# biod/sambamba

Measured on NVIDIA H100. Metric: bam_gb_per_s_depth_base, higher is better.
Workload: dtype u32

## Files before the change

__graft_entry__.py:

```python
import os
import subprocess
import sys

ROOT = os.path.dirname(os.path.abspath(__file__))
CSRC = os.path.join(ROOT, "sambamba_b200", "csrc")
NVCC = os.environ.get("NVCC", "/usr/local/cuda/bin/nvcc")


def _run(cmd, cwd=None, quiet=False):
    r = subprocess.run(cmd, cwd=cwd, stdout=subprocess.PIPE, stderr=subprocess.STDOUT, text=True)
    if r.returncode != 0:
        sys.stderr.write(r.stdout)
        raise RuntimeError("build step failed: " + " ".join(cmd))
    if not quiet and r.stdout.strip():
        print(r.stdout.strip()[-2000:])


def _stale(target, sources):
    if not os.path.exists(target):
        return True
    t = os.path.getmtime(target)
    return any(os.path.getmtime(s) > t for s in sources if os.path.exists(s))


def build(quiet=False, load=True):
    out = os.path.join(ROOT, "sambamba_b200", "_build")
    os.makedirs(out, exist_ok=True)
    lib = os.path.join(out, "libbdepth.so")
    srcs = [os.path.join(CSRC, f) for f in ("bdepth.cu", "kernels.cuh", "mates.cuh", "filter.cuh", "regex.cuh", "host_filter.hpp", "host_regex.hpp", "launch.cuh", "inflate_core.cuh", "inflate2_core.cuh", "host_bam.hpp")] + [os.path.join(ROOT, "include", "bdepth.h"), os.path.abspath(__file__)]
    if _stale(lib, srcs):
        _run([NVCC, "-gencode", "arch=compute_90a,code=sm_90a", "-O3", "-lineinfo", "-std=c++17",
              "-Xcompiler", "-fPIC,-Wall,-Wno-unused-function,-Wno-unknown-pragmas", "-shared", "-o", lib, os.path.join(CSRC, "bdepth.cu"), "-lcudart", "-ldl"], quiet=quiet)
    cli_src = os.path.join(CSRC, "cli.cpp")
    cli = os.path.join(out, "sambamba-depth-b200")
    if os.path.exists(cli_src) and _stale(cli, [cli_src, lib]):
        _run(["g++", "-O2", "-g", "-std=c++17", "-Wall", "-o", cli, cli_src, "-L" + out, "-lbdepth", "-Wl,-rpath,$ORIGIN"], quiet=quiet)
    _run(["make", "-s", "-C", os.path.join(ROOT, "oracle")], quiet=quiet)
    tb = os.path.join(ROOT, "tools", "_build")
    os.makedirs(tb, exist_ok=True)
    if _stale(os.path.join(tb, "bamgen"), [os.path.join(ROOT, "tools", "bamgen.c")]):
        _run(["gcc", "-O2", "-g", "-o", os.path.join(tb, "bamgen"), os.path.join(ROOT, "tools", "bamgen.c"), "-lz", "-lpthread", "-lm"], quiet=quiet)
    fso = os.path.join(ROOT, "tools", "flagstat_oracle.c")
    if _stale(os.path.join(tb, "flagstat_oracle"), [fso]) or _stale(os.path.join(tb, "libflagstat_oracle.so"), [fso]):
        _run(["gcc", "-O2", "-g", "-Wall", "-std=gnu11", "-DORACLE_MAIN", "-o", os.path.join(tb, "flagstat_oracle"), fso, "-lz", "-lpthread"], quiet=quiet)
        _run(["gcc", "-O2", "-g", "-Wall", "-std=gnu11", "-fPIC", "-shared", "-o", os.path.join(tb, "libflagstat_oracle.so"), fso, "-lz", "-lpthread"], quiet=quiet)
    vco = os.path.join(ROOT, "tools", "view_count_oracle.c")
    if _stale(os.path.join(tb, "view_count_oracle"), [vco]) or _stale(os.path.join(tb, "libview_count_oracle.so"), [vco]):
        _run(["gcc", "-O2", "-g", "-Wall", "-std=gnu11", "-DORACLE_MAIN", "-o", os.path.join(tb, "view_count_oracle"), vco, "-lz", "-lm"], quiet=quiet)
        _run(["gcc", "-O2", "-g", "-Wall", "-std=gnu11", "-fPIC", "-shared", "-o", os.path.join(tb, "libview_count_oracle.so"), vco, "-lz", "-lm"], quiet=quiet)
    _run(["make", "-s", "-C", os.path.join(ROOT, "tests", "emul")], quiet=quiet)
    emul = os.path.join(ROOT, "tests", "emul")
    es = os.path.join(emul, "libemul_sam.so")
    es_srcs = [os.path.join(emul, f) for f in ("emul_sam.cpp", "cuda_shim.cpp", "cuda_shim.hpp")] + [os.path.join(CSRC, f) for f in ("kernels.cuh", "filter.cuh", "regex.cuh", "launch.cuh", "inflate_core.cuh", "inflate2_core.cuh")]
    if _stale(es, es_srcs):
        _run(["g++", "-O2", "-g", "-std=c++17", "-w", "-DBDEPTH_EMULATE_SHIM=\"" + os.path.join(emul, "cuda_shim.hpp") + "\"", "-shared", "-fPIC", "-o", es,
              os.path.join(emul, "emul_sam.cpp"), os.path.join(emul, "cuda_shim.cpp"), "-ldl"], quiet=quiet)
    if load:
        sys.path.insert(0, ROOT)
        import sambamba_b200
        sambamba_b200.load_library()


def smoke():
    sys.path.insert(0, ROOT)
    sys.path.insert(0, os.path.join(ROOT, "tests"))
    import numpy as np
    import sambamba_b200 as sb
    import helpers
    path = os.path.join(ROOT, "tests", "golden", "issue_204.bam")
    win = helpers.interesting_window(path)
    with sb.BDepth(path, device=0) as b:
        got = b.run_base(window=win)
        st = b.stats()
    want, _ = helpers.oracle_counts(path, window=win)
    assert got.shape == want.shape and np.array_equal(got, want), "GPU counters differ from the oracle"
    print("smoke ok:", {k: st[k] for k in ("n_blocks", "n_records", "n_records_pass", "covered_positions", "gpu_launches")})


if __name__ == "__main__":
    build()
    if len(sys.argv) > 1 and sys.argv[1] == "smoke":
        smoke()
```

sambamba_b200/csrc/bdepth.cu:

```cuda
#include "launch.cuh"
#include <dlfcn.h>
#include <fcntl.h>
#include <stdarg.h>
#include <stdio.h>
#include <stdlib.h>
#include <sys/mman.h>
#include <sys/stat.h>
#include <unistd.h>
#include <algorithm>
#include <chrono>
#include <map>
#include <string>
#include <vector>

#include "../../include/bdepth.h"
#include "host_bam.hpp"
#include "kernels.cuh"
#include "mates.cuh"
#include "host_filter.hpp"

using namespace bdk;

namespace {

// ... 46 lines not shown
enum RunMode { RUN_FULL = 0, RUN_INFLATE_ONLY = 1, RUN_SCAN_ONLY = 2, RUN_INDEX = 3, RUN_FLAGSTAT = 4, RUN_VIEW_COUNT = 5, RUN_VIEW_TEXT = 6 };
constexpr int RC_RETRY_WINDOW = 1;

struct NcclUid { char b[128]; };
typedef void* NcclComm;
struct NcclApi {
    bool ok = false; std::string err;
    int (*GetUniqueId)(NcclUid*) = nullptr;
    int (*CommInitRank)(NcclComm*, int, NcclUid, int) = nullptr;
    int (*CommDestroy)(NcclComm) = nullptr;
    int (*AllGather)(const void*, void*, size_t, int, NcclComm, cudaStream_t) = nullptr;
    int (*AllReduce)(const void*, void*, size_t, int, int, NcclComm, cudaStream_t) = nullptr;
    int (*Send)(const void*, size_t, int, int, NcclComm, cudaStream_t) = nullptr;
    int (*Recv)(void*, size_t, int, int, NcclComm, cudaStream_t) = nullptr;
    int (*GroupStart)() = nullptr;
    int (*GroupEnd)() = nullptr;
    const char* (*GetErrorString)(int) = nullptr;
};
constexpr int NCCL_UINT32 = 3, NCCL_UINT64 = 5, NCCL_SUM = 0;
NcclApi& nccl() {
    static NcclApi api; static bool tried = false;
    if (tried) return api;
    tried = true;
#ifdef BDEPTH_EMULATE_SHIM
    api.GetUniqueId = [](NcclUid* u) { return emu_ncclGetUniqueId(u->b); };
    api.CommInitRank = [](NcclComm* c, int w, NcclUid u, int r) { return emu_ncclCommInitRank(c, w, u.b, r); };
    api.CommDestroy = emu_ncclCommDestroy; api.AllGather = emu_ncclAllGather; api.AllReduce = emu_ncclAllReduce; api.Send = emu_ncclSend; api.Recv = emu_ncclRecv;
    api.GroupStart = emu_ncclGroupStart; api.GroupEnd = emu_ncclGroupEnd; api.GetErrorString = emu_ncclGetErrorString; api.ok = true;
    return api;
#endif
    void* lib = dlopen("libnccl.so.2", RTLD_NOW | RTLD_GLOBAL);
    if (!lib) lib = dlopen("libnccl.so", RTLD_NOW | RTLD_GLOBAL);
    if (!lib) { api.err = std::string("cannot load libnccl.so.2: ") + dlerror(); return api; }
    bool all = true;
    auto sym = [&](const char* n) { void* p = dlsym(lib, n); if (!p) { all = false; api.err = std::string("missing NCCL symbol ") + n; } return p; };
    api.GetUniqueId = (int (*)(NcclUid*))sym("ncclGetUniqueId");
    api.CommInitRank = (int (*)(NcclComm*, int, NcclUid, int))sym("ncclCommInitRank");
    api.CommDestroy = (int (*)(NcclComm))sym("ncclCommDestroy");
    api.AllGather = (int (*)(const void*, void*, size_t, int, NcclComm, cudaStream_t))sym("ncclAllGather");
    api.AllReduce = (int (*)(const void*, void*, size_t, int, int, NcclComm, cudaStream_t))sym("ncclAllReduce");
    api.Send = (int (*)(const void*, size_t, int, int, NcclComm, cudaStream_t))sym("ncclSend");
    api.Recv = (int (*)(void*, size_t, int, int, NcclComm, cudaStream_t))sym("ncclRecv");
    api.GroupStart = (int (*)())sym("ncclGroupStart");
    api.GroupEnd = (int (*)())sym("ncclGroupEnd");
    api.GetErrorString = (const char* (*)(int))sym("ncclGetErrorString");
    api.ok = all;
    return api;
}

}

struct bdepth {
    const uint8_t* file = nullptr; size_t file_len = 0; bool mapped = false; int fd = -1;
    std::vector<HostBlock> blocks; uint64_t total_u = 0;
    bool lazy = false, framed_all = true; size_t framed_off = 0;
    BamHeader hdr; BaiIndex bai; bool has_index = false;
    int device = 0; int n_sm = 0;
    int mapq_gt = 0; uint32_t flag_reject = 0x600; uint32_t minq = 0;
    std::vector<bdepth_region> regions;
    int rank = 0, world = 1;
    NcclComm comm = nullptr; bool have_uid = false; NcclUid uid{};
    uint64_t own_lo = 0, own_hi = 0;
    bool bai_window_ok = true;
    bool combined = false;
    bool fix_mates = false;
    bool k1lz_v12 = false;
    bool k1lz_flat = false;
    int k1h_variant = -1;
    bool k1_onephase = false;
    bool k3_pre = false;
    bool k3_tile = true;
    bool has_fprog = false; FilterProg fprog; DevBuf fprog_d;
    DevBuf m_hash, m_flag, m_flt, m_ctl;
    uint32_t S = 1;
    DevBuf rg_ids, rg_offs, rg_samp;
    DevBuf text[2], text_tiles, text_offs, text_zero, text_samp, present;
    int coll_pending = 0;
    bool want_presence = false;
    uint64_t batch_u = 6ull << 30;
    uint64_t chunk_blocks = 13 * 32 * 16;
    bool shard_ready = false;
    size_t blk_lo = 0, blk_hi = 0; int64_t entry0 = 0; uint64_t limit_abs_u = 0;
    uint64_t zone_lin_lo = UINT64_MAX;
    uint64_t own_lo_abs_u = 0;
    bool sparse_ok = true;
    bool sparse_on = false;
    std::vector<HostBlock> vblocks; std::vector<int32_t> seg_entry ; std::vector<uint32_t> seg_limit ;
    DevBuf anchors_idx, anchors_val, chunk_limit;
    cudaStream_t s_main = nullptr, s_copy = nullptr, s_d2h = nullptr;
    cudaEvent_t ev[32] = {};
    DevBuf comp2[2];
    cudaStream_t s_k1[16] = {};
    std::vector<cudaEvent_t> chunk_ev[2], k1_ev;
    std::vector<size_t> chunk_end[2];
    bool staged = false; uint64_t staged_file_off = 0;
    DevBuf tok, lits, aux, segi, littab;
    DevBuf comp, descs, status, ubuf, chunk_start, entry, exitb, count, slot_base, slots, rec_base, walk_list;
    DevBuf soa_start, soa_span, soa_meta, soa_off, soa_ncl, soa_lseq, long_list, tile_first, tile_lo, counts, ref_len_d, ref_lin0_d, scan_stats, ref_has, ref_has_all, flt_d, lead_list, misc;
    uint64_t cnt_base = 0, win_len = 0;
    void* pinned = nullptr; size_t pinned_cap = 0;
    HostScratch hs;
    std::vector<uint32_t> ref_has_host;
    struct SegSet { bool on = false; uint32_t n = 0; bool has_min = false, has_u = false; uint64_t ext_max = 0; DevBuf s, e, pmax, id, reads, minstart, bases_reads, mbases, ustart, da, dac, db, dthr, dbases, dcov, dscr; } seg;
    struct IndexSet { DevBuf lin, lin_len, lin_base, lin_cap, n_mapped, n_unmapped, carry, ctl, runs, excs; std::vector<uint32_t> base, cap; std::vector<IndexRun> h_runs; std::vector<IndexExc> h_excs; uint64_t n_lin = 0; } ix;
    std::vector<uint8_t> built_bai;
    DevBuf fs; uint64_t fs_host[FS_WORDS + 1] = {};
    ViewSel vsel{}; DevBuf vc, vc_reg, vc_prog; uint64_t vc_host[2] = {};
    struct ViewText {
        bdepth_text_cb cb = nullptr; void* user = nullptr;
        DevBuf names, len, off, tiles, ctl, cut_r, cut_o, slot[2];
        char* host = nullptr; size_t cap = 0;
        bool pend[2] = {false, false}; size_t pend_len[2] = {0, 0}; int next = 0;
        uint64_t issued = 0;
        float ms_fmt = 0, ms_d2h = 0;
        SamTab tab{};
    } vt;
    std::vector<bdepth*> extra;
    bool accum = false;
    bool force_window = false;
    bdepth_stats st{}; std::string err;
};

namespace {

int fail(bdepth* h, int code, const char* fmt, ...) {
    char buf[1024]; va_list ap; va_start(ap, fmt); vsnprintf(buf, sizeof buf, fmt, ap); va_end(ap);
    if (h) h->err = buf; else g_open_error = buf;
    return code;
}
#define NK(call) do { int r__ = (call); if (r__ != 0) return fail(h, BDEPTH_ERR_NCCL, "NCCL error at %s:%d: %s", __FILE__, __LINE__, nccl().GetErrorString ? nccl().GetErrorString(r__) : "?"); } while (0)
#define CK(call) do { cudaError_t e__ = (call); if (e__ != cudaSuccess) return fail(h, BDEPTH_ERR_CUDA, "CUDA error %s at %s:%d: %s", cudaGetErrorName(e__), __FILE__, __LINE__, cudaGetErrorString(e__)); } while (0)

int ensure_pinned(bdepth* h, size_t n) {
    if (n <= h->pinned_cap) return 0;
    if (h->pinned) cudaFreeHost(h->pinned);
    h->hs.release();
    h->pinned = nullptr; h->pinned_cap = 0;
    CK(cudaMallocHost(&h->pinned, n));
    h->pinned_cap = n;
    return 0;
}

int init_device(bdepth* h) {
    int n = 0; cudaError_t e = cudaGetDeviceCount(&n);
    if (e != cudaSuccess || n <= 0) return fail(h, BDEPTH_ERR_CUDA, "no CUDA device available (%s); libbdepth has no CPU fallback", cudaGetErrorString(e));
    if (h->device < 0 || h->device >= n) return fail(h, BDEPTH_ERR_ARG, "device %d out of range (%d devices)", h->device, n);
    CK(cudaSetDevice(h->device));
    CK(cudaDeviceGetAttribute(&h->n_sm, cudaDevAttrMultiProcessorCount, h->device));
    if (!h->s_main) { CK(cudaStreamCreateWithFlags(&h->s_main, cudaStreamNonBlocking)); CK(cudaStreamCreateWithFlags(&h->s_copy, cudaStreamNonBlocking)); CK(cudaStreamCreateWithFlags(&h->s_d2h, cudaStreamNonBlocking)); for (auto& ks : h->s_k1) CK(cudaStreamCreateWithFlags(&ks, cudaStreamNonBlocking)); for (auto& e2 : h->ev) CK(cudaEventCreate(&e2)); }
    CK(cudaFuncSetAttribute(k1_inflate, cudaFuncAttributeMaxDynamicSharedMemorySize, K1_SMEM));
    CK(cudaFuncSetAttribute(k1_fallback, cudaFuncAttributeMaxDynamicSharedMemorySize, K1_SMEM));
    CK(cudaFuncSetAttribute(k1_huff<false, 4>, cudaFuncAttributePreferredSharedMemoryCarveout, cudaSharedmemCarveoutMaxShared)); CK(cudaFuncSetAttribute(k1_huff<false, 6>, cudaFuncAttributePreferredSharedMemoryCarveout, cudaSharedmemCarveoutMaxShared));
    CK(cudaFuncSetAttribute(k1_huff<true, 5>, cudaFuncAttributePreferredSharedMemoryCarveout, cudaSharedmemCarveoutMaxShared)); CK(cudaFuncSetAttribute(k1_huff<true, 4>, cudaFuncAttributePreferredSharedMemoryCarveout, cudaSharedmemCarveoutMaxShared));
    { const char* e = getenv("BDEPTH_K1H_VARIANT"); h->k1h_variant = e ? atoi(e) : -1; }
    { const char* e = getenv("BDEPTH_K3"); h->k3_tile = !(e && !strcmp(e, "gather")); }
    CK(cudaFuncSetAttribute(k3_tile<false>, cudaFuncAttributeMaxDynamicSharedMemorySize, (int)K3T_SMEM)); CK(cudaFuncSetAttribute(k3_tile<true>, cudaFuncAttributeMaxDynamicSharedMemorySize, (int)K3T_SMEM));
    { const char* e = getenv("BDEPTH_K1LZ"); h->k1lz_flat = e && !strcmp(e, "flat"); h->k1lz_v12 = e && !strcmp(e, "v12"); }
    { const char* e = getenv("BDEPTH_K1_ONEPHASE"); h->k1_onephase = e && atoi(e) == 1; }
    { const char* e = getenv("BDEPTH_K3_PREFETCH"); h->k3_pre = !e || atoi(e) != 0; }
    return 0;
}

int inflate_blocks_to_host(bdepth* h, size_t b0, size_t b1, std::vector<uint8_t>& out) {
    size_t nb = b1 - b0; if (!nb) { out.clear(); return 0; }
    uint64_t f0 = h->blocks[b0].coff & ~3ull, f1 = h->blocks[b1 - 1].coff + h->blocks[b1 - 1].bsize;
    uint64_t ulen = h->blocks[b1 - 1].uoff + h->blocks[b1 - 1].isize - h->blocks[b0].uoff;
    CK(h->comp.ensure(f1 - f0 + 256)); CK(h->descs.ensure(nb * sizeof(BlockDesc))); CK(h->status.ensure(nb * sizeof(int))); CK(h->ubuf.ensure(CARRY_MAX + ulen + 256));
    std::vector<BlockDesc> d(nb);
    for (size_t i = 0; i < nb; i++) { const HostBlock& b = h->blocks[b0 + i]; d[i] = BlockDesc{b.coff + b.cdata_off - f0, b.uoff - h->blocks[b0].uoff, b.csize, b.isize}; }
    CK(cudaMemcpyAsync(h->comp.p, h->file + f0, f1 - f0, cudaMemcpyHostToDevice, h->s_main));
    CK(cudaMemsetAsync((uint8_t*)h->comp.p + (f1 - f0), 0, 128, h->s_main));
    CK(cudaMemcpyAsync(h->descs.p, d.data(), nb * sizeof(BlockDesc), cudaMemcpyHostToDevice, h->s_main));
    BD_LAUNCH((unsigned)((nb + 32 * K1_WARPS - 1) / (32 * K1_WARPS)), 32 * K1_WARPS, K1_SMEM, h->s_main, k1_inflate)(h->comp.as<uint32_t>(), h->descs.as<BlockDesc>(), (uint32_t)nb, h->ubuf.as<uint8_t>() + CARRY_MAX, h->status.as<int>());
    CK(cudaGetLastError());
    std::vector<int> stt(nb); out.resize(ulen);
    CK(cudaMemcpyAsync(stt.data(), h->status.p, nb * sizeof(int), cudaMemcpyDeviceToHost, h->s_main));
    CK(cudaMemcpyAsync(out.data(), h->ubuf.as<uint8_t>() + CARRY_MAX, ulen, cudaMemcpyDeviceToHost, h->s_main));
    CK(cudaStreamSynchronize(h->s_main));
    h->st.gpu_launches += 1;
    for (size_t i = 0; i < nb; i++) if (stt[i]) return fail(h, BDEPTH_ERR_FORMAT, "DEFLATE error %d in BGZF block at offset %llu", stt[i], (unsigned long long)h->blocks[b0 + i].coff);
    return 0;
}

int frame_more(bdepth* h, size_t more) {
    if (h->framed_all) return 0;
    bool eof = false;
    std::string e = frame_bgzf(h->file, h->file_len, &h->framed_off, &h->total_u, more, UINT64_MAX, h->blocks, &eof);
    if (!e.empty()) return fail(h, BDEPTH_ERR_FORMAT, "%s", e.c_str());
    if (eof) h->framed_all = true;
    return 0;
}
int ensure_all_blocks(bdepth* h) { return frame_more(h, SIZE_MAX); }

int finish_open(bdepth* h) {
    h->blocks.clear(); h->total_u = 0; h->framed_off = 0; h->framed_all = false;
    { int rcf = frame_more(h, h->lazy ? 4 : SIZE_MAX); if (rcf) return rcf; }
    if (h->blocks.empty()) return fail(h, BDEPTH_ERR_FORMAT, "Invalid file format: expected BAM\\1");
    int rc = init_device(h); if (rc) return rc;
    size_t nb = std::min<size_t>(4, h->blocks.size());
    for (;;) {
        std::vector<uint8_t> u; rc = inflate_blocks_to_host(h, 0, nb, u); if (rc) return rc;
        std::string perr; int pr = parse_bam_header(u.data(), u.size(), h->hdr, perr);
        if (pr == 0) break;
        if (pr < 0) return fail(h, BDEPTH_ERR_FORMAT, "%s", perr.c_str());
        if (nb == h->blocks.size() && !h->framed_all) { rc = frame_more(h, nb * 3); if (rc) return rc; }
        if (nb == h->blocks.size()) return fail(h, BDEPTH_ERR_FORMAT, "truncated BAM header");
        nb = std::min(h->blocks.size(), nb * 4);
    }
    size_t nref = h->hdr.ref_len.size();
    CK(h->ref_len_d.ensure((nref + 1) * 4)); CK(h->ref_lin0_d.ensure((nref + 1) * 8));
    if (nref) { CK(cudaMemcpy(h->ref_len_d.p, h->hdr.ref_len.data(), nref * 4, cudaMemcpyHostToDevice)); CK(cudaMemcpy(h->ref_lin0_d.p, h->hdr.ref_lin0.data(), nref * 8, cudaMemcpyHostToDevice)); }
    return 0;
}

std::vector<uint64_t> shard_candidates(const BaiIndex& bai) {
    std::vector<uint64_t> vos;
    for (auto& v : bai.ioffsets) for (uint64_t x : v) if (x) vos.push_back(x);
    std::sort(vos.begin(), vos.end()); vos.erase(std::unique(vos.begin(), vos.end()), vos.end());
    return vos;
}
uint64_t shard_cut_voffset(const std::vector<uint64_t>& vos, uint64_t file_len, int k, int world) {
    uint64_t target = (uint64_t)((__uint128_t)file_len * (unsigned)k / (unsigned)world);
    auto it = std::lower_bound(vos.begin(), vos.end(), target << 16);
    return it == vos.end() ? UINT64_MAX : *it;
}

int prepare_shard(bdepth* h) {
    if (h->shard_ready) return 0;
    { int rcf = ensure_all_blocks(h); if (rcf) return rcf; }
    const auto& B = h->blocks;
    auto block_of_u = [&](uint64_t u) { size_t lo = 0, hi = B.size(); while (lo + 1 < hi) { size_t m = (lo + hi) / 2; if (B[m].uoff <= u) lo = m; else hi = m; } return lo; };
    auto block_of_c = [&](uint64_t c) { size_t lo = 0, hi = B.size(); while (lo + 1 < hi) { size_t m = (lo + hi) / 2; if (B[m].coff <= c) lo = m; else hi = m; } return lo; };
    uint64_t start_u = h->hdr.first_rec_off, end_u = h->total_u;
    if (h->world > 1) {
        if (!h->bai.valid) return fail(h, BDEPTH_ERR_NOINDEX, "sharding needs the BAI linear index");
        std::vector<uint64_t> vos = shard_candidates(h->bai);
        auto cut = [&](int k) -> uint64_t {
            if (k <= 0) return h->hdr.first_rec_off;
            if (k >= h->world) return h->total_u;
            uint64_t vo = shard_cut_voffset(vos, h->file_len, k, h->world);
            if (vo == UINT64_MAX) return h->total_u;
            size_t b = block_of_c(vo >> 16);
            if (B[b].coff != (vo >> 16)) return h->total_u;
            uint64_t u = B[b].uoff + (vo & 0xFFFF);
            return u < h->hdr.first_rec_off ? h->hdr.first_rec_off : u;
        };
        start_u = cut(h->rank); end_u = cut(h->rank + 1);
        if (end_u < start_u) end_u = start_u;
    }
    if (start_u >= h->total_u) { h->blk_lo = h->blk_hi = B.size(); h->entry0 = 0; h->limit_abs_u = h->total_u; h->shard_ready = true; return 0; }
    h->blk_lo = block_of_u(start_u); h->entry0 = (int64_t)(start_u - B[h->blk_lo].uoff);
    h->limit_abs_u = end_u; h->own_lo_abs_u = start_u;
    if (end_u >= h->total_u) h->blk_hi = B.size();
    else h->blk_hi = std::min(B.size(), block_of_u(end_u) + 1 + (h->fix_mates ? MATE_ZONE_BLOCKS : SHARD_EXTRA_BLOCKS));
    h->zone_lin_lo = UINT64_MAX;
    if (h->world > 1 && h->rank > 0) {
        std::vector<uint8_t> u; int rc = inflate_blocks_to_host(h, h->blk_lo, std::min(B.size(), h->blk_lo + 2), u); if (rc) return rc;
        const uint64_t o = (uint64_t)h->entry0;
        if (o + 12 <= u.size()) {
            int32_t ref = (int32_t)h_rd32(u.data() + o + 4), pos = (int32_t)h_rd32(u.data() + o + 8);
            if (ref >= 0 && (size_t)ref < h->bai.ioffsets.size() && pos >= 0) {
                const auto& lin = h->bai.ioffsets[ref]; size_t w = (size_t)pos >> 14;
                uint64_t vo = w < lin.size() ? lin[w] : 0;
                if (vo) {
                    size_t b = block_of_c(vo >> 16);
                    if (B[b].coff != (vo >> 16)) return fail(h, BDEPTH_ERR_FORMAT, "fix-mate-overlaps on several ranks: the linear index does not match the file");
                    uint64_t zu = B[b].uoff + (vo & 0xFFFF);
                    if (zu < h->hdr.first_rec_off) zu = h->hdr.first_rec_off;
                    if (zu < start_u) { h->blk_lo = block_of_u(zu); h->entry0 = (int64_t)(zu - B[h->blk_lo].uoff); }
                    h->zone_lin_lo = h->hdr.ref_lin0[ref] + ((uint64_t)w << 14);
                }
            }
        }
    }
    h->shard_ready = true;
    return 0;
}

struct Emitter {
    bdepth* h; bdepth_tile_cb cb; void* user;
    struct Range { uint64_t a, b; };
    std::vector<Range> ranges; size_t ri = 0; uint64_t pos = 0; bool started = false;
    uint64_t lo_clip = 0, hi_clip = UINT64_MAX;
    struct Slot { uint64_t a = 0, b = 0; } slot[2];
    int head = 0, inflight = 0;
    uint64_t d2h_bytes = 0;
    size_t chunk() const { return EMIT_CHUNK / h->S; }
    int issue(int si, uint64_t a, uint64_t b) {
        const int NP = N_PLANES * (int)h->S; const size_t CH = chunk();
        uint32_t* dst = (uint32_t*)h->pinned + (size_t)si * EMIT_CHUNK * N_PLANES;
        uint64_t wa = std::max(a, h->cnt_base), wb = std::min(b, h->cnt_base + h->win_len);
        if (wa >= wb || wa > a || wb < b) for (int pl = 0; pl < NP; pl++) memset(dst + (size_t)pl * CH, 0, (b - a) * 4);
        if (wa < wb) for (int pl = 0; pl < NP; pl++) CK(cudaMemcpyAsync(dst + (size_t)pl * CH + (wa - a), h->counts.as<uint32_t>() + (uint64_t)pl * h->win_len + (wa - h->cnt_base), (wb - wa) * 4, cudaMemcpyDeviceToHost, h->s_d2h));
        CK(cudaEventRecord(h->ev[8 + si], h->s_d2h));
        slot[si].a = a; slot[si].b = b; d2h_bytes += (b - a) * NP * 4;
        return 0;
    }
    int deliver_oldest() {
        int si = (head + 2 - inflight) & 1;
        CK(cudaEventSynchronize(h->ev[8 + si]));
        inflight--;
        if (!cb) return 0;
        const uint32_t* src = (const uint32_t*)h->pinned + (size_t)si * EMIT_CHUNK * N_PLANES;
        uint64_t a = slot[si].a, bnd = slot[si].b; const size_t nref = h->hdr.ref_len.size();
        size_t ref = std::upper_bound(h->hdr.ref_lin0.begin(), h->hdr.ref_lin0.end(), a) - h->hdr.ref_lin0.begin() - 1;
        while (a < bnd && ref < nref) {
// ... 1718 lines not shown
```

sambamba_b200/csrc/kernels.cuh:

```cuda
#pragma once
#include "launch.cuh"
#include <stdint.h>
#include "inflate_core.cuh"
#include "inflate2_core.cuh"
#include "filter.cuh"

namespace bdk {

constexpr int TILE_POS = 1024;
constexpr uint32_t SPAN_SHORT = 1024;
constexpr int N_PLANES = 7;
constexpr int64_t ENTRY_NONE = (int64_t)0x8080808080808080ull;
constexpr int ENTRY_NONE_BYTE = 0x80;

struct BlockDesc {
    uint64_t coff;
    uint64_t uoff;
    uint32_t csize;
    uint32_t isize;
    uint64_t tok_off;
};
BD_HD uint32_t tok_cap_of(uint32_t isize) { return isize / 4u + 16u; }
struct BlockAux { uint32_t n_tok, n_seg, n_lit, pad; };
BD_HD uint64_t lit_off_of(uint64_t uoff, uint64_t block_index) { return (uoff & ~15ull) + 16ull * block_index; }

constexpr int K1_WARPS = 13;
constexpr int K1_SMEM = K1_WARPS * SMEM_BYTES_PER_WARP;
__global__ void __launch_bounds__(K1_WARPS * 32, 1) k1_inflate(const uint32_t* __restrict__ comp, const BlockDesc* __restrict__ blocks,
                                                               uint32_t n_blocks, uint8_t* __restrict__ u, int* __restrict__ status) {
    BD_DYN_SMEM(uint32_t, smem);
    uint32_t lane = threadIdx.x & 31, warp = threadIdx.x >> 5;
    uint32_t b = (blockIdx.x * K1_WARPS + warp) * 32u + lane;
    uint32_t scratch[96];
    const bool active = b < n_blocks;
    BlockDesc d = active ? blocks[b] : BlockDesc{0, 0, 0, 0, 0};
    uint32_t* wbase = smem + warp * (SMEM_BYTES_PER_WARP / 4);
    SmemTab tab{wbase + lane, (uint32_t)__cvta_generic_to_shared(wbase + T_WORDS * 32) + lane * 16, (uint32_t)__cvta_generic_to_shared(wbase + T_FAR * 32 + lane)};
    ByteOut out{u};
    int rc = inflate_block(tab, comp, d.coff, d.csize, out, d.uoff, d.isize, scratch, active);
    if (active) status[b] = rc;
}


constexpr int K1H_WARPS = 4;
template <bool LIMS> constexpr int k1h_smem() { return K1H_WARPS * (H_SMEM_BYTES_PER_WARP + (LIMS ? H_LIM_BYTES_PER_WARP : 0)); }
template <bool LIMS, int MINB>
__global__ void __launch_bounds__(K1H_WARPS * 32, MINB) k1_huff(const uint32_t* __restrict__ comp, const BlockDesc* __restrict__ blocks, uint32_t n_blocks, uint32_t blk0,
                                                                int* __restrict__ status, uint32_t* __restrict__ tok, uint8_t* __restrict__ lits, BlockAux* __restrict__ aux,
                                                                uint32_t* __restrict__ seg_info, uint8_t* __restrict__ lit_tab) {
    BD_DYN_SMEM(uint32_t, smem);
    uint32_t lane = threadIdx.x & 31, warp = threadIdx.x >> 5;
    uint32_t b = (blockIdx.x * K1H_WARPS + warp) * 32u + lane;
    uint32_t scratch[96];
    const bool active = b < n_blocks;
    BlockDesc d = active ? blocks[b] : BlockDesc{0, 0, 0, 0, 0};
    constexpr int PER_WARP = (H_SMEM_BYTES_PER_WARP + (LIMS ? H_LIM_BYTES_PER_WARP : 0)) / 4;
    uint32_t* wbase = smem + warp * PER_WARP;
    uint32_t* limb = wbase + H_WORDS * 32 + (32 * RING_BYTES_PER_LANE) / 4;
    SmemTab2 tab{wbase + lane, limb + lane * 4, (uint32_t)__cvta_generic_to_shared(wbase + H_WORDS * 32) + lane * 16};
    HuffOut ho{tok + d.tok_off, tok_cap_of(d.isize), lits + lit_off_of(d.uoff, (uint64_t)blk0 + b), lit_tab + (size_t)b * (MAX_SEG * 256), seg_info + (size_t)b * MAX_SEG};
    uint32_t n_tok = 0, n_seg = 0, n_lit = 0;
    int rc = huff_phase<SmemTab2, LIMS>(tab, comp, d.coff, d.csize, d.isize, scratch, ho, n_tok, n_seg, n_lit, active);
    if (active) { status[b] = rc; aux[b] = BlockAux{n_tok, n_seg, n_lit, 0u}; }
}

__device__ __forceinline__ uint32_t ld_u32_any(const uint8_t* p) {
    uintptr_t a = reinterpret_cast<uintptr_t>(p); const uint32_t* w = reinterpret_cast<const uint32_t*>(a & ~uintptr_t(3));
    return __funnelshift_r(w[0], w[1], (uint32_t)(a & 3) * 8);
}
constexpr int K1L_WARPS = 8;
#ifndef BDEPTH_EMULATE_SHIM
__device__ __forceinline__ uint32_t warp_max_u32(uint32_t v) { return __reduce_max_sync(0xFFFFFFFFu, v); }
#else
static inline uint32_t warp_max_u32(uint32_t v) { return ~__reduce_min_sync(0xFFFFFFFFu, ~v); }
static inline bool emu_k1lz_warp() { static const bool on = getenv("BDEPTH_EMU_K1LZ_WARP") && atoi(getenv("BDEPTH_EMU_K1LZ_WARP")) == 1; return on; }
#endif
template <bool COMPACT>
__global__ void __launch_bounds__(K1L_WARPS * 32, 6) k1_lz(const BlockDesc* __restrict__ blocks, uint32_t n_blocks, uint32_t blk0, uint8_t* __restrict__ u, int* __restrict__ status,
                                                        const uint32_t* __restrict__ tok, const uint8_t* __restrict__ lits, const BlockAux* __restrict__ aux,
                                                        const uint32_t* __restrict__ seg_info, const uint8_t* __restrict__ lit_tab) {
    __shared__ uint32_t s_tab[K1L_WARPS][64];
    __shared__ uint32_t s_il[K1L_WARPS][33], s_dl[K1L_WARPS][33];
    const uint32_t lane = threadIdx.x & 31, warp = threadIdx.x >> 5;
    const uint32_t b = blockIdx.x * K1L_WARPS + warp;
    if (b >= n_blocks || status[b] != INF_OK) return;
    const BlockDesc d = blocks[b]; const BlockAux ax = aux[b];
    uint8_t* const ub = u + d.uoff;
    const uint8_t* const lt = lits + lit_off_of(d.uoff, (uint64_t)blk0 + b);
    const uint32_t* const sgi = seg_info + (size_t)b * MAX_SEG;
    const uint8_t* const ltab = lit_tab + (size_t)b * (MAX_SEG * 256);
#ifdef BDEPTH_EMULATE_SHIM
    if (!emu_k1lz_warp()) {
        if (lane == 0) { int rcs = lz_phase_serial(ub, d.isize, tok + d.tok_off, ax.n_tok, lt, ax.n_lit, ltab, sgi, ax.n_seg); if (rcs) status[b] = rcs; }
        return;
    }
#endif
    const uint8_t* const tb = reinterpret_cast<const uint8_t*>(s_tab[warp]);
    uint32_t sg = 0, seg_hi = ax.n_seg > 1 ? (sgi[1] & 0x7FFFFFFFu) : 0xFFFFFFFFu; bool seg_raw = ax.n_seg == 0 || (sgi[0] & SEG_RAW);
    if (!seg_raw) { const uint32_t* tg = reinterpret_cast<const uint32_t*>(ltab); s_tab[warp][lane] = tg[lane]; s_tab[warp][lane + 32] = tg[lane + 32]; }
    __syncwarp();
    const uint32_t* tk = tok + d.tok_off;
    uint32_t base = 0, lbase = 0;
    int err = INF_OK;
    for (uint32_t g = 0; g < ax.n_tok; g += 32) {
        const uint32_t t = g + lane < ax.n_tok ? tk[g + lane] : TOK_NOMATCH;
        const uint32_t lit = t & 0xFFu, len = (t >> 31) ? 0u : ((t >> 8) & 0xFFu) + 3u, dist = ((t >> 16) & 0x7FFFu) + 1u;
        uint32_t incl = lit + len, il = lit;
#pragma unroll
        for (int o = 1; o < 32; o <<= 1) { uint32_t v = __shfl_up_sync(0xFFFFFFFFu, incl, o), w = __shfl_up_sync(0xFFFFFFFFu, il, o); if ((int)lane >= o) { incl += v; il += w; } }
        const uint32_t tot = __shfl_sync(0xFFFFFFFFu, incl, 31), totl = __shfl_sync(0xFFFFFFFFu, il, 31);
        const uint32_t dlit = base + incl - len - lit, dst = dlit + lit;
        {
            const bool far = len && dist > dst;
            if (__ballot_sync(0xFFFFFFFFu, far)) { err = INF_ERR_DIST; break; }
            if (base + tot > d.isize || lbase + totl > ax.n_lit) { err = INF_ERR_OVERRUN; break; }
        }
        if (totl) {
            while (sg + 1 < ax.n_seg && lbase >= seg_hi) {
                sg++; seg_hi = sg + 1 < ax.n_seg ? (sgi[sg + 1] & 0x7FFFFFFFu) : 0xFFFFFFFFu; seg_raw = (sgi[sg] & SEG_RAW) != 0;
                __syncwarp();
                if (!seg_raw) { const uint32_t* tg = reinterpret_cast<const uint32_t*>(ltab + sg * 256u); s_tab[warp][lane] = tg[lane]; s_tab[warp][lane + 32] = tg[lane + 32]; }
                __syncwarp();
            }
            const bool one_seg = lbase + totl <= seg_hi;
            int n_ent = 32;
            if (COMPACT) {
                const unsigned has_l = __ballot_sync(0xFFFFFFFFu, lit != 0);
                if (lit) { const uint32_t e = __popc(has_l & ((1u << lane) - 1u)); s_il[warp][e] = il; s_dl[warp][e] = dlit; }
                n_ent = __popc(has_l);
            } else { s_il[warp][lane] = il; s_dl[warp][lane] = dlit; }
            __syncwarp();
            for (uint32_t j0 = 4 * lane; j0 < totl; j0 += 128) {
                const uint32_t w = ld_u32_any(lt + lbase + j0);
                int lo = 0, hi = n_ent - 1;
                while (lo < hi) { int mid = (lo + hi) >> 1; if (s_il[warp][mid] > j0) hi = mid; else lo = mid + 1; }
                uint32_t tend = s_il[warp][lo], tbeg = lo ? s_il[warp][lo - 1] : 0u, tdst = s_dl[warp][lo];
#pragma unroll
                for (uint32_t bq = 0; bq < 4; bq++) {
                    const uint32_t j = j0 + bq;
                    if (j >= totl) break;
                    if (COMPACT) { if (j >= tend) { lo++; tbeg = tend; tend = s_il[warp][lo]; tdst = s_dl[warp][lo]; } }
                    else while (j >= tend) { lo++; tbeg = tend; tend = s_il[warp][lo]; tdst = s_dl[warp][lo]; }
                    const uint32_t r = (w >> (8 * bq)) & 0xFFu;
                    uint32_t v;
                    if (one_seg) v = seg_raw ? r : (uint32_t)tb[r];
                    else {
                        uint32_t s2 = sg; while (s2 + 1 < ax.n_seg && lbase + j >= (sgi[s2 + 1] & 0x7FFFFFFFu)) s2++;
                        v = (sgi[s2] & SEG_RAW) ? r : (uint32_t)ltab[s2 * 256u + r];
                    }
                    ub[tdst + (j - tbeg)] = (uint8_t)v;
                }
            }
            __syncwarp();
        }
        {
            const uint32_t need = len ? ((dst - dist + len < dst) ? dst - dist + len : dst) : 0u;
            uint8_t* dp = ub + dst; const uint8_t* sp = dp - dist;
            unsigned pending = __ballot_sync(0xFFFFFFFFu, len != 0);
            while (pending) {
                const uint32_t ready = __shfl_sync(0xFFFFFFFFu, dst, __ffs(pending) - 1);
                const bool go = ((pending >> lane) & 1u) && need <= ready;
                const uint32_t ml = warp_max_u32(go ? len : 0u);
                for (uint32_t k = 0; k < ml; k += 4) {
                    if (!go || k >= len) continue;
                    const uint32_t n = len - k < 4u ? len - k : 4u;
                    if (dist >= 4) {
                        const uint32_t w = ld_u32_any(sp + k);
                        dp[k] = (uint8_t)w;
                        if (n > 1) dp[k + 1] = (uint8_t)(w >> 8);
                        if (n > 2) dp[k + 2] = (uint8_t)(w >> 16);
                        if (n > 3) dp[k + 3] = (uint8_t)(w >> 24);
                    } else for (uint32_t q = 0; q < n; q++) dp[k + q] = sp[k + q];
                }
                pending &= ~__ballot_sync(0xFFFFFFFFu, go);
                __syncwarp();
            }
        }
        base += tot; lbase += totl;
    }
    if (!err && (base != d.isize || lbase != ax.n_lit)) err = INF_ERR_SHORT;
    if (err && lane == 0) status[b] = err;
}

__global__ void __launch_bounds__(K1L_WARPS * 32) k1_lz_flat(const BlockDesc* __restrict__ blocks, uint32_t n_blocks, uint32_t blk0, uint8_t* __restrict__ u, int* __restrict__ status,
                                                             const uint32_t* __restrict__ tok, const uint8_t* __restrict__ lits, const BlockAux* __restrict__ aux,
                                                             const uint32_t* __restrict__ seg_info, const uint8_t* __restrict__ lit_tab) {
    __shared__ uint32_t s_tab[K1L_WARPS][64];
    __shared__ uint32_t s_end[K1L_WARPS][32], s_il[K1L_WARPS][32], s_dist[K1L_WARPS][32];
    const uint32_t lane = threadIdx.x & 31, warp = threadIdx.x >> 5;
    const uint32_t b = blockIdx.x * K1L_WARPS + warp;
    if (b >= n_blocks || status[b] != INF_OK) return;
    const BlockDesc d = blocks[b]; const BlockAux ax = aux[b];
    uint8_t* const ub = u + d.uoff;
    const uint8_t* const lt = lits + lit_off_of(d.uoff, (uint64_t)blk0 + b);
    const uint32_t* const sgi = seg_info + (size_t)b * MAX_SEG;
    const uint8_t* const ltab = lit_tab + (size_t)b * (MAX_SEG * 256);
    const uint8_t* const tb = reinterpret_cast<const uint8_t*>(s_tab[warp]);
    uint32_t sg = 0, seg_hi = ax.n_seg > 1 ? (sgi[1] & 0x7FFFFFFFu) : 0xFFFFFFFFu; bool seg_raw = ax.n_seg == 0 || (sgi[0] & SEG_RAW);
    if (!seg_raw) { const uint32_t* tg = reinterpret_cast<const uint32_t*>(ltab); s_tab[warp][lane] = tg[lane]; s_tab[warp][lane + 32] = tg[lane + 32]; }
    __syncwarp();
    const uint32_t* tk = tok + d.tok_off;
    uint32_t base = 0, lbase = 0;
    int err = INF_OK;
    for (uint32_t g = 0; g < ax.n_tok; g += 32) {
        const uint32_t t = g + lane < ax.n_tok ? tk[g + lane] : TOK_NOMATCH;
        const uint32_t lit = t & 0xFFu, len = (t >> 31) ? 0u : ((t >> 8) & 0xFFu) + 3u, dist = ((t >> 16) & 0x7FFFu) + 1u;
        uint32_t incl = lit + len, il = lit;
#pragma unroll
        for (int o = 1; o < 32; o <<= 1) { uint32_t v = __shfl_up_sync(0xFFFFFFFFu, incl, o), w = __shfl_up_sync(0xFFFFFFFFu, il, o); if ((int)lane >= o) { incl += v; il += w; } }
        const uint32_t tot = __shfl_sync(0xFFFFFFFFu, incl, 31), totl = __shfl_sync(0xFFFFFFFFu, il, 31);
        const uint32_t tstart = incl - len - lit;
        {
            const bool far = len && dist > base + tstart + lit;
            if (__ballot_sync(0xFFFFFFFFu, far)) { err = INF_ERR_DIST; break; }
            if (base + tot > d.isize || lbase + totl > ax.n_lit) { err = INF_ERR_OVERRUN; break; }
        }
        if (totl) {
            while (sg + 1 < ax.n_seg && lbase >= seg_hi) {
                sg++; seg_hi = sg + 1 < ax.n_seg ? (sgi[sg + 1] & 0x7FFFFFFFu) : 0xFFFFFFFFu; seg_raw = (sgi[sg] & SEG_RAW) != 0;
                __syncwarp();
                if (!seg_raw) { const uint32_t* tg = reinterpret_cast<const uint32_t*>(ltab + sg * 256u); s_tab[warp][lane] = tg[lane]; s_tab[warp][lane + 32] = tg[lane + 32]; }
                __syncwarp();
            }
        }
        const bool one_seg = lbase + totl <= seg_hi;
        auto literal = [&](uint32_t li) -> uint32_t {
            const uint32_t r = lt[li];
            if (one_seg) return seg_raw ? r : (uint32_t)tb[r];
            uint32_t s2 = sg; while (s2 + 1 < ax.n_seg && li >= (sgi[s2 + 1] & 0x7FFFFFFFu)) s2++;
            return (sgi[s2] & SEG_RAW) ? r : (uint32_t)ltab[s2 * 256u + r];
        };
        s_end[warp][lane] = incl; s_il[warp][lane] = il; s_dist[warp][lane] = dist;
        __syncwarp();
        const bool real = lit + len != 0;
        for (uint32_t o0 = 0; o0 < tot; o0 += 32) {
            const uint32_t mbits = __reduce_or_sync(0xFFFFFFFFu, (real && tstart >= o0 && tstart < o0 + 32) ? (1u << (tstart - o0)) : 0u);
            const uint32_t first = (uint32_t)__popc(__ballot_sync(0xFFFFFFFFu, real && tstart <= o0)) - 1u;
            const uint32_t o = o0 + lane;
            if (o < tot) {
                uint32_t i = first + (uint32_t)__popc(mbits & ((2u << lane) - 1u) & ~1u);
                uint32_t ts = i ? s_end[warp][i - 1] : 0u, lb = i ? s_il[warp][i - 1] : 0u, li = s_il[warp][i] - lb, off = o - ts;
                uint32_t v;
                if (off < li) v = literal(lbase + lb + off);
                else {
                    uint32_t k = off - li, dd = s_dist[warp][i], ms = base + ts + li;
                    uint32_t s = ms - dd + (dd <= k ? k % dd : k);
                    bool done = false; v = 0;
                    while (s >= base) {
                        const uint32_t so = s - base;
                        int lo = 0, hi = (int)i;
                        while (lo < hi) { int mid = (lo + hi) >> 1; if (s_end[warp][mid] > so) hi = mid; else lo = mid + 1; }
                        ts = lo ? s_end[warp][lo - 1] : 0u; lb = lo ? s_il[warp][lo - 1] : 0u; li = s_il[warp][lo] - lb; off = so - ts;
                        if (off < li) { v = literal(lbase + lb + off); done = true; break; }
                        k = off - li; dd = s_dist[warp][lo]; ms = base + ts + li;
                        s = ms - dd + (dd <= k ? k % dd : k);
                    }
                    if (!done) v = ub[s];
                }
                ub[base + o] = (uint8_t)v;
            }
        }
        base += tot; lbase += totl;
        __syncwarp();
    }
    if (!err && (base != d.isize || lbase != ax.n_lit)) err = INF_ERR_SHORT;
    if (err && lane == 0) status[b] = err;
}

__global__ void __launch_bounds__(K1_WARPS * 32, 1) k1_fallback(const uint32_t* __restrict__ comp, const BlockDesc* __restrict__ blocks,
                                                                uint32_t n_blocks, uint8_t* __restrict__ u, int* __restrict__ status) {
    BD_DYN_SMEM(uint32_t, smem);
    uint32_t lane = threadIdx.x & 31, warp = threadIdx.x >> 5;
    uint32_t b = (blockIdx.x * K1_WARPS + warp) * 32u + lane;
    uint32_t scratch[96];
    const bool active = b < n_blocks && status[b] == INF_FALLBACK;
#ifndef BDEPTH_EMULATE_SHIM
    if (!__any_sync(0xFFFFFFFFu, active)) return;
#endif
    BlockDesc d = active ? blocks[b] : BlockDesc{0, 0, 0, 0, 0};
    uint32_t* wbase = smem + warp * (SMEM_BYTES_PER_WARP / 4);
    SmemTab tab{wbase + lane, (uint32_t)__cvta_generic_to_shared(wbase + T_WORDS * 32) + lane * 16, (uint32_t)__cvta_generic_to_shared(wbase + T_FAR * 32 + lane)};
    ByteOut out{u};
    int rc = inflate_block(tab, comp, d.coff, d.csize, out, d.uoff, d.isize, scratch, active);
    if (active) status[b] = rc;
}

__device__ __forceinline__ uint32_t ldu32(const uint8_t* p) {
    uintptr_t a = reinterpret_cast<uintptr_t>(p);
    const uint32_t* w = reinterpret_cast<const uint32_t*>(a & ~uintptr_t(3));
    uint32_t lo = __ldg(w), hi = __ldg(w + 1);
    return __funnelshift_r(lo, hi, (uint32_t)(a & 3) * 8);
}
__device__ __forceinline__ uint32_t ldu16(const uint8_t* p) { return ldu32(p) & 0xFFFFu; }

struct ScanParams {
    const uint8_t* u;
    int64_t u_begin;
    int64_t u_end;
    int n_ref;
    const uint32_t* ref_len;
    const uint64_t* ref_lin0;
};

__device__ __forceinline__ bool plausible_record(const ScanParams& sp, int64_t o, int64_t* next) {
    if (o + 36 > sp.u_end) return false;
    const uint8_t* p = sp.u + o;
    uint32_t bs = ldu32(p);
    if (bs < 32u || bs > (1u << 28)) return false;
    int32_t ref = (int32_t)ldu32(p + 4), pos = (int32_t)ldu32(p + 8);
    if (ref < -1 || ref >= sp.n_ref || pos < -1) return false;
    if (ref >= 0 && (uint32_t)pos > sp.ref_len[ref]) return false;
    uint32_t l_name = p[12];
    uint32_t n_cigar = ldu16(p + 16);
    int32_t l_seq = (int32_t)ldu32(p + 20);
    int32_t nref = (int32_t)ldu32(p + 24), npos = (int32_t)ldu32(p + 28);
    if (l_name < 1 || l_seq < 0 || nref < -1 || nref >= sp.n_ref || npos < -1) return false;
    uint64_t need = 32ull + l_name + 4ull * n_cigar + ((uint64_t)l_seq + 1) / 2 + (uint64_t)l_seq;
    if (need > bs) return false;
    int64_t nul = o + 36 + l_name - 1;
    if (nul < sp.u_end && sp.u[nul] != 0) return false;
    *next = o + 4 + (int64_t)bs;
    return true;
}

__global__ void k2_guess_entries(ScanParams sp, const int64_t* __restrict__ chunk_start, uint32_t n_chunks, int64_t* __restrict__ entry) {
    uint32_t warp = (blockIdx.x * blockDim.x + threadIdx.x) >> 5, lane = threadIdx.x & 31;
    if (warp >= n_chunks) return;
    if (warp == 0) return;
    int64_t c0 = chunk_start[warp], c1 = chunk_start[warp + 1];
    int64_t found = ENTRY_NONE;
    for (int64_t base = c0; base < c1; base += 32) {
        int64_t o = base + lane, nx = 0;
// ... 1252 lines not shown
```

Measured before the change: 45.50.

## Stage LZ77 decode output through per-warp shared-memory ring window

```diff
diff --git a/__graft_entry__.py b/__graft_entry__.py
--- a/__graft_entry__.py
+++ b/__graft_entry__.py
@@ -55,6 +55,11 @@
     if _stale(es, es_srcs):
         _run(["g++", "-O2", "-g", "-std=c++17", "-w", "-DBDEPTH_EMULATE_SHIM=\"" + os.path.join(emul, "cuda_shim.hpp") + "\"", "-shared", "-fPIC", "-o", es,
               os.path.join(emul, "emul_sam.cpp"), os.path.join(emul, "cuda_shim.cpp"), "-ldl"], quiet=quiet)
+    ek = os.path.join(emul, "libemul_k1lz.so")
+    ek_srcs = [os.path.join(emul, f) for f in ("emul_k1lz.cpp", "cuda_shim.cpp", "cuda_shim.hpp")] + [os.path.join(CSRC, f) for f in ("kernels.cuh", "filter.cuh", "regex.cuh", "launch.cuh", "inflate_core.cuh", "inflate2_core.cuh")]
+    if _stale(ek, ek_srcs):
+        _run(["g++", "-O1", "-g", "-std=c++17", "-w", "-DBDEPTH_EMULATE_SHIM=\"" + os.path.join(emul, "cuda_shim.hpp") + "\"", "-shared", "-fPIC", "-o", ek,
+              os.path.join(emul, "emul_k1lz.cpp"), os.path.join(emul, "cuda_shim.cpp"), "-ldl"], quiet=quiet)
     if load:
         sys.path.insert(0, ROOT)
         import sambamba_b200
diff --git a/sambamba_b200/csrc/bdepth.cu b/sambamba_b200/csrc/bdepth.cu
--- a/sambamba_b200/csrc/bdepth.cu
+++ b/sambamba_b200/csrc/bdepth.cu
@@ -222,6 +222,7 @@
     CK(cudaFuncSetAttribute(k1_fallback, cudaFuncAttributeMaxDynamicSharedMemorySize, K1_SMEM));
     CK(cudaFuncSetAttribute(k1_huff<false, 4>, cudaFuncAttributePreferredSharedMemoryCarveout, cudaSharedmemCarveoutMaxShared)); CK(cudaFuncSetAttribute(k1_huff<false, 6>, cudaFuncAttributePreferredSharedMemoryCarveout, cudaSharedmemCarveoutMaxShared));
     CK(cudaFuncSetAttribute(k1_huff<true, 5>, cudaFuncAttributePreferredSharedMemoryCarveout, cudaSharedmemCarveoutMaxShared)); CK(cudaFuncSetAttribute(k1_huff<true, 4>, cudaFuncAttributePreferredSharedMemoryCarveout, cudaSharedmemCarveoutMaxShared));
+    CK(cudaFuncSetAttribute(k1_lz<true>, cudaFuncAttributePreferredSharedMemoryCarveout, cudaSharedmemCarveoutMaxShared)); CK(cudaFuncSetAttribute(k1_lz<false>, cudaFuncAttributePreferredSharedMemoryCarveout, cudaSharedmemCarveoutMaxShared));
     { const char* e = getenv("BDEPTH_K1H_VARIANT"); h->k1h_variant = e ? atoi(e) : -1; }
     { const char* e = getenv("BDEPTH_K3"); h->k3_tile = !(e && !strcmp(e, "gather")); }
     CK(cudaFuncSetAttribute(k3_tile<false>, cudaFuncAttributeMaxDynamicSharedMemorySize, (int)K3T_SMEM)); CK(cudaFuncSetAttribute(k3_tile<true>, cudaFuncAttributeMaxDynamicSharedMemorySize, (int)K3T_SMEM));
diff --git a/sambamba_b200/csrc/kernels.cuh b/sambamba_b200/csrc/kernels.cuh
--- a/sambamba_b200/csrc/kernels.cuh
+++ b/sambamba_b200/csrc/kernels.cuh
@@ -1,6 +1,7 @@
 #pragma once
 #include "launch.cuh"
 #include <stdint.h>
+#include <type_traits>
 #include "inflate_core.cuh"
 #include "inflate2_core.cuh"
 #include "filter.cuh"
@@ -69,6 +70,25 @@
     return __funnelshift_r(w[0], w[1], (uint32_t)(a & 3) * 8);
 }
 constexpr int K1L_WARPS = 8;
+constexpr uint32_t K1L_WIN = 4096;
+__device__ __forceinline__ uint32_t ring_ld32(const uint32_t* r, uint32_t i) {
+    i &= K1L_WIN - 1;
+    return __funnelshift_r(r[i >> 2], r[((i >> 2) + 1) & (K1L_WIN / 4 - 1)], (i & 3) * 8);
+}
+__device__ __forceinline__ void ring_flush(const uint32_t* r, uint8_t* ub, uint32_t ua, uint32_t lo, uint32_t hi, uint32_t lane) {
+    const uint8_t* rb = reinterpret_cast<const uint8_t*>(r);
+    const uint32_t l0 = min(hi, lo + ((0u - (ua + lo)) & 15u)), part = (ua + hi) & 15u, l1 = hi - l0 >= part ? hi - part : l0;
+    if (lane < l0 - lo) ub[lo + lane] = rb[(ua + lo + lane) & (K1L_WIN - 1)];
+    if (lane < hi - l1) ub[l1 + lane] = rb[(ua + l1 + lane) & (K1L_WIN - 1)];
+    for (uint32_t p = l0 + 16 * lane; p < l1; p += 512) {
+        const uint32_t i = ((ua + p) & (K1L_WIN - 1)) >> 2;
+#ifndef BDEPTH_EMULATE_SHIM
+        *reinterpret_cast<uint4*>(ub + p) = make_uint4(r[i], r[i + 1], r[i + 2], r[i + 3]);
+#else
+        for (int q = 0; q < 4; q++) for (int c = 0; c < 4; c++) ub[p + 4 * q + c] = (uint8_t)(r[i + q] >> (8 * c));
+#endif
+    }
+}
 #ifndef BDEPTH_EMULATE_SHIM
 __device__ __forceinline__ uint32_t warp_max_u32(uint32_t v) { return __reduce_max_sync(0xFFFFFFFFu, v); }
 #else
@@ -76,16 +96,20 @@
 static inline bool emu_k1lz_warp() { static const bool on = getenv("BDEPTH_EMU_K1LZ_WARP") && atoi(getenv("BDEPTH_EMU_K1LZ_WARP")) == 1; return on; }
 #endif
 template <bool COMPACT>
-__global__ void __launch_bounds__(K1L_WARPS * 32, 6) k1_lz(const BlockDesc* __restrict__ blocks, uint32_t n_blocks, uint32_t blk0, uint8_t* __restrict__ u, int* __restrict__ status,
+__global__ void __launch_bounds__(K1L_WARPS * 32, 5) k1_lz(const BlockDesc* __restrict__ blocks, uint32_t n_blocks, uint32_t blk0, uint8_t* __restrict__ u, int* __restrict__ status,
                                                         const uint32_t* __restrict__ tok, const uint8_t* __restrict__ lits, const BlockAux* __restrict__ aux,
                                                         const uint32_t* __restrict__ seg_info, const uint8_t* __restrict__ lit_tab) {
     __shared__ uint32_t s_tab[K1L_WARPS][64];
     __shared__ uint32_t s_il[K1L_WARPS][33], s_dl[K1L_WARPS][33];
+    __shared__ uint4 s_win[K1L_WARPS][K1L_WIN / 16];
     const uint32_t lane = threadIdx.x & 31, warp = threadIdx.x >> 5;
     const uint32_t b = blockIdx.x * K1L_WARPS + warp;
     if (b >= n_blocks || status[b] != INF_OK) return;
     const BlockDesc d = blocks[b]; const BlockAux ax = aux[b];
     uint8_t* const ub = u + d.uoff;
+    uint32_t* const rw = reinterpret_cast<uint32_t*>(s_win[warp]);
+    uint8_t* const rb = reinterpret_cast<uint8_t*>(rw);
+    const uint32_t ua = (uint32_t)reinterpret_cast<uintptr_t>(ub);
     const uint8_t* const lt = lits + lit_off_of(d.uoff, (uint64_t)blk0 + b);
     const uint32_t* const sgi = seg_info + (size_t)b * MAX_SEG;
     const uint8_t* const ltab = lit_tab + (size_t)b * (MAX_SEG * 256);
@@ -101,6 +125,7 @@
     __syncwarp();
     const uint32_t* tk = tok + d.tok_off;
     uint32_t base = 0, lbase = 0;
+    uint32_t wm = 0;
     int err = INF_OK;
     for (uint32_t g = 0; g < ax.n_tok; g += 32) {
         const uint32_t t = g + lane < ax.n_tok ? tk[g + lane] : TOK_NOMATCH;
@@ -115,69 +140,102 @@
             if (__ballot_sync(0xFFFFFFFFu, far)) { err = INF_ERR_DIST; break; }
             if (base + tot > d.isize || lbase + totl > ax.n_lit) { err = INF_ERR_OVERRUN; break; }
         }
-        if (totl) {
-            while (sg + 1 < ax.n_seg && lbase >= seg_hi) {
-                sg++; seg_hi = sg + 1 < ax.n_seg ? (sgi[sg + 1] & 0x7FFFFFFFu) : 0xFFFFFFFFu; seg_raw = (sgi[sg] & SEG_RAW) != 0;
+        const bool win = tot + 16u <= K1L_WIN;
+        if (!win) { ring_flush(rw, ub, ua, wm, base, lane); wm = base; __syncwarp(); }
+        auto group = [&](auto win_c) {
+            constexpr bool WIN = decltype(win_c)::value;
+            if (totl) {
+                while (sg + 1 < ax.n_seg && lbase >= seg_hi) {
+                    sg++; seg_hi = sg + 1 < ax.n_seg ? (sgi[sg + 1] & 0x7FFFFFFFu) : 0xFFFFFFFFu; seg_raw = (sgi[sg] & SEG_RAW) != 0;
+                    __syncwarp();
+                    if (!seg_raw) { const uint32_t* tg = reinterpret_cast<const uint32_t*>(ltab + sg * 256u); s_tab[warp][lane] = tg[lane]; s_tab[warp][lane + 32] = tg[lane + 32]; }
+                    __syncwarp();
+                }
+                const bool one_seg = lbase + totl <= seg_hi;
+                int n_ent = 32;
+                if (COMPACT) {
+                    const unsigned has_l = __ballot_sync(0xFFFFFFFFu, lit != 0);
+                    if (lit) { const uint32_t e = __popc(has_l & ((1u << lane) - 1u)); s_il[warp][e] = il; s_dl[warp][e] = dlit; }
+                    n_ent = __popc(has_l);
+                } else { s_il[warp][lane] = il; s_dl[warp][lane] = dlit; }
                 __syncwarp();
-                if (!seg_raw) { const uint32_t* tg = reinterpret_cast<const uint32_t*>(ltab + sg * 256u); s_tab[warp][lane] = tg[lane]; s_tab[warp][lane + 32] = tg[lane + 32]; }
+                for (uint32_t j0 = 4 * lane; j0 < totl; j0 += 128) {
+                    const uint32_t w = ld_u32_any(lt + lbase + j0);
+                    int lo = 0, hi = n_ent - 1;
+                    while (lo < hi) { int mid = (lo + hi) >> 1; if (s_il[warp][mid] > j0) hi = mid; else lo = mid + 1; }
+                    uint32_t tend = s_il[warp][lo], tbeg = lo ? s_il[warp][lo - 1] : 0u, tdst = s_dl[warp][lo];
+#pragma unroll
+                    for (uint32_t bq = 0; bq < 4; bq++) {
+                        const uint32_t j = j0 + bq;
+                        if (j >= totl) break;
+                        if (COMPACT) { if (j >= tend) { lo++; tbeg = tend; tend = s_il[warp][lo]; tdst = s_dl[warp][lo]; } }
+                        else while (j >= tend) { lo++; tbeg = tend; tend = s_il[warp][lo]; tdst = s_dl[warp][lo]; }
+                        const uint32_t r = (w >> (8 * bq)) & 0xFFu;
+                        uint32_t v;
+                        if (one_seg) v = seg_raw ? r : (uint32_t)tb[r];
+                        else {
+                            uint32_t s2 = sg; while (s2 + 1 < ax.n_seg && lbase + j >= (sgi[s2 + 1] & 0x7FFFFFFFu)) s2++;
+                            v = (sgi[s2] & SEG_RAW) ? r : (uint32_t)ltab[s2 * 256u + r];
+                        }
+                        const uint32_t p = tdst + (j - tbeg);
+                        if (WIN) rb[(ua + p) & (K1L_WIN - 1)] = (uint8_t)v; else ub[p] = (uint8_t)v;
+                    }
+                }
                 __syncwarp();
             }
-            const bool one_seg = lbase + totl <= seg_hi;
-            int n_ent = 32;
-            if (COMPACT) {
-                const unsigned has_l = __ballot_sync(0xFFFFFFFFu, lit != 0);
-                if (lit) { const uint32_t e = __popc(has_l & ((1u << lane) - 1u)); s_il[warp][e] = il; s_dl[warp][e] = dlit; }
-                n_ent = __popc(has_l);
-            } else { s_il[warp][lane] = il; s_dl[warp][lane] = dlit; }
-            __syncwarp();
-            for (uint32_t j0 = 4 * lane; j0 < totl; j0 += 128) {
-                const uint32_t w = ld_u32_any(lt + lbase + j0);
-                int lo = 0, hi = n_ent - 1;
-                while (lo < hi) { int mid = (lo + hi) >> 1; if (s_il[warp][mid] > j0) hi = mid; else lo = mid + 1; }
-                uint32_t tend = s_il[warp][lo], tbeg = lo ? s_il[warp][lo - 1] : 0u, tdst = s_dl[warp][lo];
-#pragma unroll
-                for (uint32_t bq = 0; bq < 4; bq++) {
-                    const uint32_t j = j0 + bq;
-                    if (j >= totl) break;
-                    if (COMPACT) { if (j >= tend) { lo++; tbeg = tend; tend = s_il[warp][lo]; tdst = s_dl[warp][lo]; } }
-                    else while (j >= tend) { lo++; tbeg = tend; tend = s_il[warp][lo]; tdst = s_dl[warp][lo]; }
-                    const uint32_t r = (w >> (8 * bq)) & 0xFFu;
-                    uint32_t v;
-                    if (one_seg) v = seg_raw ? r : (uint32_t)tb[r];
-                    else {
-                        uint32_t s2 = sg; while (s2 + 1 < ax.n_seg && lbase + j >= (sgi[s2 + 1] & 0x7FFFFFFFu)) s2++;
-                        v = (sgi[s2] & SEG_RAW) ? r : (uint32_t)ltab[s2 * 256u + r];
+            {
+                const uint32_t need = len ? ((dst - dist + len < dst) ? dst - dist + len : dst) : 0u;
+                const uint32_t s = dst - dist;
+                const uint32_t rlo = base + tot > K1L_WIN ? base + tot - K1L_WIN : 0u;
+                const bool from_ring = WIN && s >= rlo, whole = !WIN || from_ring || s + len <= rlo;
+                unsigned pending = __ballot_sync(0xFFFFFFFFu, len != 0);
+                while (pending) {
+                    const uint32_t ready = __shfl_sync(0xFFFFFFFFu, dst, __ffs(pending) - 1);
+                    const bool go = ((pending >> lane) & 1u) && need <= ready;
+                    const uint32_t ml = warp_max_u32(go ? len : 0u);
+                    for (uint32_t k = 0; k < ml; k += 4) {
+                        if (!go || k >= len) continue;
+                        const uint32_t n = len - k < 4u ? len - k : 4u;
+                        if (dist >= 4 && whole) {
+                            const uint32_t w = from_ring ? ring_ld32(rw, ua + s + k) : ld_u32_any(ub + s + k);
+                            if (WIN) {
+                                const uint32_t p = (ua + dst + k) & (K1L_WIN - 1);
+                                if (p <= K1L_WIN - 4) {
+                                    uint8_t* dp = rb + p;
+                                    dp[0] = (uint8_t)w;
+                                    if (n > 1) dp[1] = (uint8_t)(w >> 8);
+                                    if (n > 2) dp[2] = (uint8_t)(w >> 16);
+                                    if (n > 3) dp[3] = (uint8_t)(w >> 24);
+                                } else for (uint32_t q = 0; q < n; q++) rb[(p + q) & (K1L_WIN - 1)] = (uint8_t)(w >> (8 * q));
+                            } else {
+                                uint8_t* dp = ub + dst + k;
+                                dp[0] = (uint8_t)w;
+                                if (n > 1) dp[1] = (uint8_t)(w >> 8);
+                                if (n > 2) dp[2] = (uint8_t)(w >> 16);
+                                if (n > 3) dp[3] = (uint8_t)(w >> 24);
+                            }
+                        } else for (uint32_t q = 0; q < n; q++) {
+                            const uint32_t p = s + k + q, v = WIN && p >= rlo ? rb[(ua + p) & (K1L_WIN - 1)] : ub[p];
+                            if (WIN) rb[(ua + dst + k + q) & (K1L_WIN - 1)] = (uint8_t)v; else ub[dst + k + q] = (uint8_t)v;
+                        }
                     }
-                    ub[tdst + (j - tbeg)] = (uint8_t)v;
+                    pending &= ~__ballot_sync(0xFFFFFFFFu, go);
+                    __syncwarp();
                 }
             }
-            __syncwarp();
-        }
-        {
-            const uint32_t need = len ? ((dst - dist + len < dst) ? dst - dist + len : dst) : 0u;
-            uint8_t* dp = ub + dst; const uint8_t* sp = dp - dist;
-            unsigned pending = __ballot_sync(0xFFFFFFFFu, len != 0);
-            while (pending) {
-                const uint32_t ready = __shfl_sync(0xFFFFFFFFu, dst, __ffs(pending) - 1);
-                const bool go = ((pending >> lane) & 1u) && need <= ready;
-                const uint32_t ml = warp_max_u32(go ? len : 0u);
-                for (uint32_t k = 0; k < ml; k += 4) {
-                    if (!go || k >= len) continue;
-                    const uint32_t n = len - k < 4u ? len - k : 4u;
-                    if (dist >= 4) {
-                        const uint32_t w = ld_u32_any(sp + k);
-                        dp[k] = (uint8_t)w;
-                        if (n > 1) dp[k + 1] = (uint8_t)(w >> 8);
-                        if (n > 2) dp[k + 2] = (uint8_t)(w >> 16);
-                        if (n > 3) dp[k + 3] = (uint8_t)(w >> 24);
-                    } else for (uint32_t q = 0; q < n; q++) dp[k + q] = sp[k + q];
-                }
-                pending &= ~__ballot_sync(0xFFFFFFFFu, go);
-                __syncwarp();
-            }
-        }
+        };
+        if (win) group(std::true_type{}); else group(std::false_type{});
         base += tot; lbase += totl;
-    }
+        if (win) {
+            const uint32_t r = (ua + base) & 15u, hi = base - wm >= r ? base - r : wm;
+            ring_flush(rw, ub, ua, wm, hi, lane); wm = hi;
+        } else {
+            for (uint32_t p = (base > K1L_WIN ? max(base - K1L_WIN, wm) : wm) + lane; p < base; p += 32) rb[(ua + p) & (K1L_WIN - 1)] = ub[p];
+            wm = base;
+        }
+        __syncwarp();
+    }
+    ring_flush(rw, ub, ua, wm, base, lane);
     if (!err && (base != d.isize || lbase != ax.n_lit)) err = INF_ERR_SHORT;
     if (err && lane == 0) status[b] = err;
 }
```

After: 46.58 (median of 6 runs). 2.4% higher.
